# MarvinChung/simple-implementation-of-structure-from-motion-and-multi-view-stereo-by-python

Measured on AMD Instinct MI355X. Metric: candidate patches/sec NCC-scored (640×480, 48 views) at 1/2/4/8 MI355X; % HBM roofline, higher is better.
Workload: dtype u8; 1 GPU; dinoRing 48x640x480, one expansion sweep of 1048576 candidates per GPU, 11x11 NCC (wid=5) vs all views, MIN_NCC 0.7, one GPU (no exchange); global_batch=1048576, wid=5, views=48, outputs=per candidate: xy + one record [mask word, avg] (|V| = popcount), parallelism=single GPU

## Files before the change

include/mvs_amd.h:

```cpp
#ifndef MVS_AMD_H
#define MVS_AMD_H

#include <stdint.h>

#ifdef __cplusplus
extern "C" {
#endif

#define MVS_OK 0
#define MVS_E_ARG (-1)
#define MVS_E_HIP (-2)
#define MVS_E_UNSUPPORTED (-3)
#define MVS_E_NOMEM (-4)
#define MVS_E_DIVZERO (-5)

typedef struct mvs_ctx mvs_ctx;
typedef struct mvs_stage_result mvs_stage_result;
typedef struct mvs_stage mvs_stage;

const char* mvs_version(void);

int mvs_ctx_create(int device, int V, int H, int W, const uint8_t* rgb, const double* K,
                   const double* R, const double* t, const double* Rp, mvs_ctx** out);
void mvs_ctx_destroy(mvs_ctx* ctx);
// ... 19 lines not shown
                        const uint64_t* mask, const int32_t* count, const double* avg,
                        const double* c, const double* nrm, uint8_t* alive, int64_t* stats);
int mvs_pack_accepted(mvs_ctx* ctx, int64_t n, int64_t offset, const int32_t* d_count,
                      const uint64_t* d_mask, const double* d_c, int vlb, int64_t cap, int64_t* d_out,
                      void* stream);
int mvs_proxy_copy(void* d_dst, const void* d_src, int64_t bytes, int workgroups, void* stream);
int mvs_set_scorer_grid(mvs_ctx* ctx, int workgroups);
int mvs_kernel_timing(mvs_ctx* ctx, int enable);
int mvs_kernel_time(mvs_ctx* ctx, double* total_ms, int64_t* launches);
const char* mvs_timed_kernel(const mvs_ctx* ctx);
int64_t mvs_exact_hits(mvs_ctx* ctx);
int mvs_stream_retiring(mvs_ctx* ctx, void* stream);

int mvs_scorer_stats(mvs_ctx* ctx, int64_t* out);

int mvs_ncc_windows(int64_t n, int npx, const uint8_t* d_a, const uint8_t* d_b, double thr,
                    int force_exact, double* d_ncc, uint8_t* d_pass, void* stream);

int mvs_stage_run(mvs_ctx* ctx, int64_t n_tracks, const int64_t* track_off,
                  const int32_t* obs_view, const float* obs_xy, int cell_size, double scale,
                  int wid, int64_t max_pops, mvs_stage_result** out);
int64_t mvs_stage_count(const mvs_stage_result* res, int which);
int mvs_stage_rows(const mvs_stage_result* res, int which, double* rows);
int mvs_stage_rows_device(const mvs_stage_result* res, int which, double* d_rows, void* stream);
int mvs_stage_stats(const mvs_stage_result* res, int64_t* stats);
int mvs_stage_times(const mvs_stage_result* res, double* times);
void mvs_stage_free(mvs_stage_result* res);

#define MVS_STAGE_FILTER_OUTLIERS 1
int mvs_exact_avg(mvs_ctx* ctx, int64_t n, const int32_t* ref, const double* xy, const uint64_t* mask,
// ... 40 lines not shown
```

simple-implementation-of-structure-from-motion-and-multi-view-stereo-by-python_amd/_lib.py:

```python
import atexit
import ctypes
import os
import weakref

import numpy as np

HERE = os.path.dirname(os.path.abspath(__file__))
LIB_PATH = os.path.join(HERE, "libmvs_amd.so")

_dp = ctypes.POINTER(ctypes.c_double)
_fp = ctypes.POINTER(ctypes.c_float)
_u8p = ctypes.POINTER(ctypes.c_uint8)
_i32p = ctypes.POINTER(ctypes.c_int32)
_i64p = ctypes.POINTER(ctypes.c_int64)
_u64p = ctypes.POINTER(ctypes.c_uint64)
_vp = ctypes.c_void_p

SIGNATURES = [
    ("mvs_version", ctypes.c_char_p, []),
    ("mvs_last_error", ctypes.c_char_p, [_vp]),
    ("mvs_ctx_create", ctypes.c_int, [ctypes.c_int, ctypes.c_int, ctypes.c_int, ctypes.c_int, _u8p,
                                      _dp, _dp, _dp, _dp, ctypes.POINTER(_vp)]),
    ("mvs_ctx_destroy", None, [_vp]),
    ("mvs_ctx_rproj", ctypes.c_int, [_vp, _dp]),
# ... 4 lines not shown
                                        ctypes.c_double, _vp, _vp, _vp, _vp, _vp]),
    ("mvs_score_device_rec", ctypes.c_int, [_vp, ctypes.c_int64, _vp, _vp, ctypes.c_int, ctypes.c_double,
                                            _vp, _vp, _vp]),
    ("mvs_score_warped", ctypes.c_int, [_vp, ctypes.c_int64, _dp, _dp, _i32p, ctypes.c_int, ctypes.c_double,
                                        ctypes.c_double, _dp, _u64p, _i32p, _dp, _dp]),
    ("mvs_score_warped_device", ctypes.c_int, [_vp, ctypes.c_int64, _vp, _vp, _vp, ctypes.c_int,
                                               ctypes.c_double, ctypes.c_double, _vp, _vp, _vp, _vp, _vp, _vp]),
    ("mvs_pack_accepted", ctypes.c_int, [_vp, ctypes.c_int64, ctypes.c_int64, _vp, _vp, _vp, ctypes.c_int,
                                         ctypes.c_int64, _vp, _vp]),
    ("mvs_set_scorer_grid", ctypes.c_int, [_vp, ctypes.c_int]),
    ("mvs_proxy_copy", ctypes.c_int, [_vp, _vp, ctypes.c_int64, ctypes.c_int, _vp]),
    ("mvs_filter_outliers", ctypes.c_int, [ctypes.c_int64, ctypes.c_int, ctypes.c_int, ctypes.c_int, _i32p,
                                           _u64p, _i32p, _dp, _dp, _dp, _u8p, _i64p]),
    ("mvs_exact_hits", ctypes.c_int64, [_vp]),
    ("mvs_scorer_stats", ctypes.c_int, [_vp, _i64p]),
    ("mvs_stream_retiring", ctypes.c_int, [_vp, _vp]),
    ("mvs_kernel_timing", ctypes.c_int, [_vp, ctypes.c_int]),
    ("mvs_kernel_time", ctypes.c_int, [_vp, ctypes.POINTER(ctypes.c_double),
                                       ctypes.POINTER(ctypes.c_int64)]),
    ("mvs_timed_kernel", ctypes.c_char_p, [_vp]),
    ("mvs_ncc_windows", ctypes.c_int, [ctypes.c_int64, ctypes.c_int, _vp, _vp, ctypes.c_double,
                                       ctypes.c_int, _vp, _vp, _vp]),
    ("mvs_stage_run", ctypes.c_int, [_vp, ctypes.c_int64, _i64p, _i32p, _fp, ctypes.c_int,
                                     ctypes.c_double, ctypes.c_int, ctypes.c_int64,
                                     ctypes.POINTER(_vp)]),
    ("mvs_stage_begin", ctypes.c_int, [_vp, ctypes.c_int64, _i64p, _i32p, _fp, ctypes.c_int,
                                       ctypes.c_double, ctypes.c_int, ctypes.c_int64, ctypes.c_int,
                                       ctypes.c_int, ctypes.POINTER(_vp)]),
    ("mvs_stage_plan", ctypes.c_int64, [_vp]),
    ("mvs_stage_record_width", ctypes.c_int, [_vp]),
# ... 189 lines not shown
        return self._h

    def rproj(self):
        out = np.empty((self.V, 9))
        check(load().mvs_ctx_rproj(self._h, _p(out, _dp)), self._h, "mvs_ctx_rproj")
        return out.reshape(self.V, 3, 3)

    def exact_hits(self):
        return int(load().mvs_exact_hits(self._h))

    def scorer_stats(self):
        out = np.zeros(3, np.int64)
        check(load().mvs_scorer_stats(self._h, _p(out, _i64p)), self._h, "mvs_scorer_stats")
        return {"direct": int(out[0]), "overflow": int(out[1]), "batches": int(out[2])}

    def rebuild(self, stream=None):
        check(load().mvs_ctx_rebuild(self._h, stream), self._h, "mvs_ctx_rebuild")

    def kernel_timing(self, enable=True, every=1):
        check(load().mvs_kernel_timing(self._h, int(every) if enable else 0), self._h, "mvs_kernel_timing")

    def kernel_time(self):
        ms = ctypes.c_double(0.0)
        k = ctypes.c_int64(0)
        check(load().mvs_kernel_time(self._h, ctypes.byref(ms), ctypes.byref(k)), self._h,
              "mvs_kernel_time")
        return ms.value, int(k.value)

    def timed_kernel(self):
        name = load().mvs_timed_kernel(self._h)
# ... 280 lines not shown
```

simple-implementation-of-structure-from-motion-and-multi-view-stereo-by-python_amd/csrc/mvs_engine.cpp:

```cpp
#include <algorithm>
#include <chrono>
#include <cfloat>
#include <cmath>
#include <cstdio>
#include <cstdlib>
#include <cstring>
#include <memory>
#include <string>
#include <vector>

#include "../../include/mvs_amd.h"
#include "mvs_internal.h"

namespace {

thread_local std::string g_err;

struct Fail {
    int code;
    std::string msg;
};

#define HIPCHK(x)                                                                         \
    do {                                                                                  \
// ... 240 lines not shown
    std::vector<uint8_t> h_rgb;
    DevBuf<uint8_t> d_rgb, d_stack, d_gv;
    DevBuf<CamDev> d_cams;
    DevBuf<int32_t> d_exact;
    DevBuf<unsigned long long> d_stats;
    SceneDev sc{};
    DevBuf<double> s_c, s_xy, s_avg;
    DevBuf<int32_t> s_ref, s_count;
    DevBuf<uint64_t> s_mask;
    DevBuf<double> w_in, w_out, w_ncc;
    DevBuf<int32_t> w_ref, w_count;
    DevBuf<uint64_t> w_mask;
    DevBuf<int32_t> t_tiles, t_cand;
    DevBuf<unsigned long long> p_ctl;
    DevBuf<int4> t_items;
    DevBuf<float> f_resp, f_dil;
    DevBuf<uint32_t> f_key, f_desc;
    DevBuf<int32_t> f_rows, f_pts, f_mom, f_best;
    int kernel_mode = 0;
    int tab_mode = 0;
    int scorer_wgs = 0;
    DevBuf<int16_t> mom_sb[MVS_MAX_WID + 1];
    DevBuf<double> mom_w[MVS_MAX_WID + 1];
    DevBuf<int32_t> mom_d[MVS_MAX_WID + 1];
    DevBuf<uint16_t> mom_flat[MVS_MAX_WID + 1];
    bool mom_ok[MVS_MAX_WID + 1] = {};
    int moments_vp() const { return V > MVS_GROUP_VIEWS ? 64 * ((V + 63) / 64) : 16 * ((V + 15) / 16); }
    MomentsDev moments(int wid) const {
        MomentsDev m{};
        m.sb = mom_sb[wid].p;
// ... 159 lines not shown
    a.xy = d_xy;
    a.mask = d_mask;
    a.count = d_count;
    a.avg = d_avg;
    a.exact_hits = ctx->d_exact.p;
    a.mstride = ctx->words();
    a.astride = 1;
    a.rec = 0;
    if (!d_count) {
        a.rec = 1;
        a.mstride = a.astride = ctx->words() + 1;
        a.avg = (double*)(d_mask + ctx->words());
    }
    const bool grouped = ctx->V > MVS_GROUP_VIEWS;
    const bool tiled = ctx->kernel_mode == 2 || (ctx->kernel_mode == 0 && n >= 2048);
    if (tiled) {
        TiledArgs t{};
        t.tw = MVS_TILE_W;
        t.th = MVS_TILE_H;
        t.ntx = (ctx->W + MVS_TILE_W - 1) / MVS_TILE_W;
        t.nty = (ctx->H + MVS_TILE_H - 1) / MVS_TILE_H;
        const int ntiles = t.ntx * t.nty;
        const int32_t* tiles_before = ctx->t_tiles.p;
        const int64_t set_words = tc_words(ntiles);
        ctx->t_tiles.ensure((size_t)(2 * set_words));
        if (ctx->t_tiles.p != tiles_before) ctx->tiles_clean_ntiles = -1;
        const int groups = grouped ? (ctx->V + MVS_GROUP_VIEWS - 1) / MVS_GROUP_VIEWS : 1;
        const int64_t mean = (n + ntiles - 1) / ntiles;
        int64_t cap = std::min<int64_t>(std::max<int64_t>(16 * mean, 1024), std::max<int64_t>(n, 64));
        cap = (cap + 63) & ~(int64_t)63;
// ... 8 lines not shown
        t.tile_count = set;
        int32_t* ctl = set + (int64_t)ntiles * kTcStride;
        t.head = ctl;
        t.fix_count = ctl + 32;
        t.n_items = ctl + 96;
        t.zero_blk = ctx->t_tiles.p + (1 - ctx->tiles_parity) * set_words;
        t.zero_words = set_words;
        t.sorted = (int2*)ctx->t_cand.p;
        t.fix_list = (int4*)(ctx->t_cand.p + 2 * (size_t)ntiles * cap);
        t.item_seg = (int)(n / std::max(t.chunk, 1) + ntiles + 2);
        ctx->t_items.ensure((size_t)kItemSegs * t.item_seg);
        t.items = ctx->t_items.p;
        t.zero_first = ctx->tiles_clean_ntiles != ntiles ? 1 : 0;
        t.grid = ctx->scorer_wgs;
        t.stats = ctx->d_stats.p;
        ctx->tiles_clean_ntiles = -1;
        hipEvent_t e0, e1;
        ctx->next_events(&e0, &e1);
        ctx->scratch_acquire(s);
        const bool tab = ctx->ensure_moments(wid, s);
        const MomentsDev mt = ctx->moments(wid);
        const int rc = mvs_launch_score_tiled(&ctx->sc, &a, &t, wid, tab ? &mt : nullptr, s, e0, e1);
        if (rc != 0) throw Fail{rc == -3 ? MVS_E_UNSUPPORTED : MVS_E_HIP, "tiled score launch failed"};
        ctx->scratch_release(s);
        if (e0) ctx->timed_name = mvs_timed_kernel_name(ctx->V, wid, tab && !grouped ? 2 : 1);
        ctx->tiles_clean_ntiles = ntiles;
        ctx->tiles_parity ^= 1;
        return;
    }
    hipEvent_t e0, e1;
    ctx->next_events(&e0, &e1);
    if (mvs_launch_score(&ctx->sc, &a, wid, s, e0, e1) != 0) throw Fail{MVS_E_HIP, "score launch failed"};
    if (e0) ctx->timed_name = mvs_timed_kernel_name(ctx->V, wid, 0);
}

void expand_device(mvs_ctx* ctx, const RecordsDev& r, const ExpandArgs& a, int wid, hipStream_t s) {
// ... 707 lines not shown
        HIPCHK(hipMemcpyAsync(ctx->d_cams.p, ctx->cams.data(), V * sizeof(CamDev), hipMemcpyHostToDevice, ctx->stream));
        ctx->d_exact.alloc(1);
        HIPCHK(hipMemsetAsync(ctx->d_exact.p, 0, sizeof(int32_t), ctx->stream));
        ctx->d_stats.alloc(4);
        HIPCHK(hipMemsetAsync(ctx->d_stats.p, 0, 4 * sizeof(unsigned long long), ctx->stream));
        HIPCHK(hipStreamSynchronize(ctx->stream));
        ctx->sc.cams = ctx->d_cams.p;
        if (const char* km = std::getenv("MVS_SCORE_KERNEL")) {
            if (!std::strcmp(km, "direct")) ctx->kernel_mode = 1;
            else if (!std::strcmp(km, "tiled")) ctx->kernel_mode = 2;
            else if (!std::strcmp(km, "mma")) ctx->tab_mode = 1;
            else if (!std::strcmp(km, "tab")) ctx->tab_mode = 2;
        }
        if (const char* sw = std::getenv("MVS_SCORER_WGS")) ctx->scorer_wgs = std::max(0, std::atoi(sw));
        if (const char* tl = std::getenv("MVS_TAB_LIMIT")) ctx->tab_limit = std::max<int64_t>(1, std::atoll(tl));
        return 0;
    });
    if (rc != 0) {
        g_err = ctx->err;
        return rc;
    }
    *out = ctx.release();
    return 0;
}

void mvs_ctx_destroy(mvs_ctx* ctx) {
    if (!ctx) return;
    (void)hipSetDevice(ctx->device);
    if (ctx->scratch_order.used || ctx->pack_order.used) (void)hipDeviceSynchronize();
    if (ctx->stream) (void)hipStreamSynchronize(ctx->stream);
// ... 250 lines not shown
        ctx->pack_order.retire((hipStream_t)stream);
        return 0;
    });
}

int mvs_scorer_stats(mvs_ctx* ctx, int64_t* out) {
    if (!ctx || !out) return set_err(ctx, Fail{MVS_E_ARG, "null argument"});
    return guarded(ctx, [&]() {
        unsigned long long h[4] = {0, 0, 0, 0};
        HIPCHK(hipMemcpyAsync(h, ctx->d_stats.p, sizeof h, hipMemcpyDeviceToHost, ctx->stream));
        HIPCHK(hipStreamSynchronize(ctx->stream));
        for (int k = 0; k < 3; ++k) out[k] = (int64_t)h[k];
        return 0;
    });
}

int mvs_ncc_windows(int64_t n, int npx, const uint8_t* d_a, const uint8_t* d_b, double thr,
                    int force_exact, double* d_ncc, uint8_t* d_pass, void* stream) {
    if (npx < 1 || npx > 128) return set_err(nullptr, Fail{MVS_E_UNSUPPORTED, "npx must be in 1..128"});
    int rc = mvs_launch_ncc_windows(n, npx, d_a, d_b, thr, force_exact, d_ncc, d_pass, (hipStream_t)stream);
    if (rc) return set_err(nullptr, Fail{MVS_E_HIP, "ncc_windows launch failed"});
    return 0;
}

int mvs_stage_run(mvs_ctx* ctx, int64_t n_tracks, const int64_t* track_off, const int32_t* obs_view,
                  const float* obs_xy, int cell_size, double scale, int wid, int64_t max_pops,
                  mvs_stage_result** out) {
    if (!ctx) return set_err(nullptr, Fail{MVS_E_ARG, "null context"});
    if (!out || n_tracks < 0 || (n_tracks > 0 && (!track_off || !obs_view || !obs_xy)) || cell_size < 1)
        return set_err(ctx, Fail{MVS_E_ARG, "bad arguments"});
// ... 447 lines not shown
```

simple-implementation-of-structure-from-motion-and-multi-view-stereo-by-python_amd/csrc/mvs_internal.h:

```cpp
#pragma once
#include <hip/hip_runtime.h>
#include <stdint.h>

#define MVS_MAX_VIEWS 256
#define MVS_MAX_WID 5

struct CamDev {
    double Rp[9];
    double t[3];
    double fx, fy, cx, cy;
    double R[9];
    double O[3];
    double C[3];
    double fbar;
    double pad[3];
};

struct SceneDev {
    int V, H, W;
    int Wq;
    int64_t row_bytes;
    const uint8_t* stack;
    const uint8_t* rgb;
    const CamDev* cams;
// ... 47 lines not shown
    int32_t* tile_count;
    int32_t* head;
    int2* sorted;
    int4* fix_list;
    int32_t* fix_count;
    int32_t* n_items;
    int item_seg;
    int32_t* zero_blk;
    int64_t zero_words;
    int groups;
    int zero_first;
    int4* items;
    int grid;
    int implicit;
    unsigned long long* stats;
};
#ifndef MVS_BIN_PER
#define MVS_BIN_PER 4
#endif
#ifndef MVS_BIN_BLOCK
#define MVS_BIN_BLOCK 1024
#endif
#define MVS_BIN_CHUNK (MVS_BIN_BLOCK * MVS_BIN_PER)
struct MomentsDev {
    int16_t* sb;
    double* w;
    int32_t* d;
    uint16_t* flat;
    int VP;
    int wid;
};
// ... 33 lines not shown
#define MVS_GROUP_VIEWS 64
#define MVS_GROUP_CHUNK 116
#ifndef MVS_ACC_PER
#define MVS_ACC_PER 8
#endif
#define MVS_ACC_CHUNK (1024 * MVS_ACC_PER)

extern "C" {
int mvs_launch_build_scene(const SceneDev* sc, const uint8_t* d_rgb, uint8_t* d_stack, uint8_t* d_gv_base,
                           hipStream_t s);
int mvs_launch_score(const SceneDev* sc, const ScoreArgs* a, int wid, hipStream_t s,
                     hipEvent_t ev0, hipEvent_t ev1);
int mvs_launch_score_warp(const SceneDev* sc, const WarpArgs* a, int wid, hipStream_t s);
int mvs_launch_score_tiled(const SceneDev* sc, const ScoreArgs* a, const TiledArgs* t, int wid,
                           const MomentsDev* mt, hipStream_t s, hipEvent_t ev0, hipEvent_t ev1);
int mvs_launch_moments(const SceneDev* sc, const MomentsDev* mt, hipStream_t s);
int mvs_launch_score_tab(const SceneDev* sc, const ScoreArgs* a, const TiledArgs* t, const MomentsDev* mt,
                         hipStream_t s);
size_t mvs_mma_lds_bytes(int V, int wid);
const char* mvs_timed_kernel_name(int V, int wid, int tiled);
int mvs_launch_expand(const SceneDev* sc, RecordsDev rec, const ExpandArgs* a, int wid,
                      hipStream_t s);
int mvs_launch_expand_geom(const SceneDev* sc, RecordsDev rec, const ExpandArgs* a, hipStream_t s);
int mvs_launch_expand_accept(RecordsDev rec, const ExpandArgs* a, hipStream_t s);
int mvs_launch_expand_ingest(RecordsDev rec, const ExpandArgs* a, int words, hipStream_t s);
int mvs_launch_pack_accepted(int64_t n, int64_t offset, const int32_t* count, const uint64_t* mask, const double* c,
                             int words, int vlb, int64_t cap, unsigned long long* ctl, int64_t* out, hipStream_t s);
int mvs_launch_proxy_copy(void* dst, const void* src, int64_t bytes, int workgroups, hipStream_t s);
int mvs_launch_ncc_windows(int64_t n, int npx, const uint8_t* a, const uint8_t* b, double thr,
                           int force_exact, double* ncc, uint8_t* pass, hipStream_t s);
// ... 19 lines not shown
```

simple-implementation-of-structure-from-motion-and-multi-view-stereo-by-python_amd/csrc/mvs_kernels.hip:

```cpp
#include <algorithm>
#include <atomic>
#include <cstdlib>
#include <utility>

#include <hipcub/hipcub.hpp>

#include "mvs_device.h"
#include "mvs_mma.h"

namespace {

template <int WID>
__device__ __noinline__ double exact_ncc_stack(const SceneDev sc, int R, int v, int q, int r) {
    constexpr int NB = 2 * WID + 1, NPX = NB * NB;
    constexpr int NW = (NB + 3) / 4, ND = NW + 1;
    const int64_t vstride = (int64_t)sc.V * 4;
    const int o = (q - WID) & 3;
    const uint8_t* p0 = sc.stack + (int64_t)(r - WID) * sc.row_bytes + (int64_t)((q - WID) >> 2) * vstride;
    auto window = [&](int view, uint32_t (&w)[NB][NW]) {
        uint32_t d[NB][ND];
#pragma unroll
        for (int row = 0; row < NB; ++row)
#pragma unroll
            for (int j = 0; j < ND; ++j)
// ... 327 lines not shown
    __syncthreads();
    if (threadIdx.x == 0) {
        int run = 0;
        for (int w = 0; w < kScanThreads / 64; ++w) { const int c = s_w[w]; s_w[w] = run; run += c; }
        s_w[kScanThreads / 64] = run;
    }
    __syncthreads();
    int slot = s_w[threadIdx.x >> 6] + incl - mine;
    for (int k = t0; k < t1; ++k) {
        const int c = min(t.tile_count[k * kTcStride], t.cap);
        for (int j = 0; j * t.chunk < c; ++j) t.items[slot++] = make_int4(k, j, 0, 0);
    }
    if (threadIdx.x < kItemSegs) t.n_items[32 * threadIdx.x] = threadIdx.x == 0 ? s_w[kScanThreads / 64] : 0;
}

template <bool LDSHIST>
__global__ __launch_bounds__(kBinBlock) void k_bin(const SceneDev sc, const ScoreArgs a,
                                                   const TiledArgs t, int wid, const MomentsDev mt) {
    extern __shared__ int32_t hist[];
    __shared__ double s_cam[16][MVS_MAX_VIEWS];
    const int words = (sc.V + 63) >> 6;
    const int64_t base = (int64_t)blockIdx.x * kBinBlock * kBinPer;
    int Rk[kBinPer];
    double ck[kBinPer][3];
#pragma unroll
    for (int k = 0; k < kBinPer; ++k) {
        const int64_t i = base + (int64_t)k * kBinBlock + threadIdx.x;
        const int64_t ii = i < a.n ? i : 0;
        Rk[k] = a.ref[ii];
        ck[k][0] = a.c[3 * ii];
        ck[k][1] = a.c[3 * ii + 1];
// ... 57 lines not shown
        }
        const int R = Rk[k], q = qk[k], r = rk[k];
        const int tx = q / MVS_TILE_W, ty = r / MVS_TILE_H;
        const int tile = ty * t.ntx + tx;
        tl[k] = tile;
        pk[k] = (q - tx * MVS_TILE_W) | ((r - ty * MVS_TILE_H) << 4) | (R << 7);
        if (LDSHIST) {
            lr[k] = atomicAdd(&hist[tile], 1);
        } else {
            lr[k] = atomicAdd(&t.tile_count[tile * kTcStride], 1);
            if (t.implicit && lr[k] > 0 && lr[k] < t.cap && lr[k] % t.chunk == 0)
                t.items[t.item_seg + atomicAdd(&t.n_items[32], 1)] = make_int4(tile, lr[k] / t.chunk, 0, 0);
        }
    }
    STAMP(t1);
    if (LDSHIST) {
        __syncthreads();
        int bs[kBinLdsTiles / kBinBlock];
#pragma unroll
        for (int j = 0; j < kBinLdsTiles / kBinBlock; ++j) {
            const int b = threadIdx.x + j * kBinBlock;
            const int c = b < t.ntiles ? hist[b] : 0;
            bs[j] = c ? atomicAdd(&t.tile_count[b * kTcStride], c) : 0;
        }
        auto bs_tile = [&](int jj) { return (int)threadIdx.x + jj * kBinBlock; };
        if (t.implicit) {
#pragma unroll
            for (int j = 0; j < kBinLdsTiles / kBinBlock; ++j) {
                const int b = bs_tile(j);
                const int c = b < t.ntiles ? hist[b] : 0;
// ... 1555 lines not shown
                         hipStream_t s, hipEvent_t ev0, hipEvent_t ev1) {
    if (a->n == 0) return 0;
    const bool grouped = sc->V > kGroupViews;
    if (t->tw != MVS_TILE_W || t->th != MVS_TILE_H || t->items == nullptr ||
        t->chunk != (grouped ? kGroupChunk : kMmaChunk) || t->groups != (grouped ? (sc->V + 63) / 64 : 1) ||
        sc->V > MVS_MAX_VIEWS)
        return -3;
    if (t->zero_first &&
        (hipMemsetAsync(t->tile_count, 0, sizeof(int32_t) * tc_words(t->ntiles), s) != hipSuccess ||
         hipMemsetAsync(t->zero_blk, 0, sizeof(int32_t) * t->zero_words, s) != hipSuccess))
        return -1;
    const int64_t per_block = (int64_t)kBinBlock * kBinPer;
    const int nbin = (int)((a->n + per_block - 1) / per_block);
    TiledArgs tv = *t;
    tv.implicit = (!grouped && mt && a->n >= (int64_t)kImplicitMean * t->ntiles) ? 1 : 0;
    const MomentsDev mflat = mt ? *mt : MomentsDev{};
    if (t->ntiles <= kBinLdsTiles)
        hipLaunchKernelGGL(k_bin<true>, dim3(nbin), dim3(kBinBlock), (size_t)t->ntiles * 4, s, *sc, *a, tv, WID, mflat);
    else
        hipLaunchKernelGGL(k_bin<false>, dim3(nbin), dim3(kBinBlock), 0, s, *sc, *a, tv, WID, mflat);
    if (!tv.implicit) hipLaunchKernelGGL(k_item_scan, dim3(1), dim3(kScanThreads), 0, s, tv);
    t = &tv;
    int rc = 0;
    {
        TimedLaunch tl(s, ev0, ev1);
        if (grouped) rc = launch_mma<WID, 4, true>(sc, a, t, mt, s);
        else if (mt) rc = mvs_launch_score_tab(sc, a, t, mt, s);
        else switch ((sc->V + 15) / 16) {
            case 1: rc = launch_mma<WID, 1, false>(sc, a, t, nullptr, s); break;
            case 2: rc = launch_mma<WID, 2, false>(sc, a, t, nullptr, s); break;
            case 3: rc = launch_mma<WID, 3, false>(sc, a, t, nullptr, s); break;
            default: rc = launch_mma<WID, 4, false>(sc, a, t, nullptr, s); break;
// ... 25 lines not shown
    return hipGetLastError() == hipSuccess ? 0 : -1;
}

int grid_for(int64_t n, int block, int cap) {
    return (int)std::max<int64_t>(1, std::min<int64_t>((n + block - 1) / block, cap));
}

}

#ifdef MVS_STAMPS
extern "C" int mvs_read_stamps(unsigned long long* out) {
    return hipMemcpyFromSymbol(out, HIP_SYMBOL(g_stamps), sizeof(g_stamps)) == hipSuccess ? 0 : -1;
}
#endif

extern "C" int mvs_launch_build_scene(const SceneDev* sc, const uint8_t* d_rgb, uint8_t* d_stack,
                                      uint8_t* d_gv_base, hipStream_t s) {
    (void)d_gv_base;
    const dim3 grid((unsigned)((sc->W + kSceneStrip - 1) / kSceneStrip), (unsigned)sc->H);
    hipLaunchKernelGGL(k_build_scene, grid, dim3(256), 0, s, *sc, d_rgb, d_stack, (uint8_t*)sc->gv);
    return hipGetLastError() == hipSuccess ? 0 : -1;
}

extern "C" int mvs_launch_score(const SceneDev* sc, const ScoreArgs* a, int wid, hipStream_t s,
                                hipEvent_t ev0, hipEvent_t ev1) {
    switch (wid) {
        case 1: return launch_score_w<1>(sc, a, s, ev0, ev1);
        case 2: return launch_score_w<2>(sc, a, s, ev0, ev1);
        case 3: return launch_score_w<3>(sc, a, s, ev0, ev1);
        case 4: return launch_score_w<4>(sc, a, s, ev0, ev1);
// ... 143 lines not shown
```

simple-implementation-of-structure-from-motion-and-multi-view-stereo-by-python_amd/csrc/mvs_score_tab.hip:

```cpp
#include <algorithm>

#include "mvs_device.h"
#include "mvs_mma.h"

namespace {

constexpr int kMomW = 32, kMomH = 16, kMomV = 16;

template <int WID, bool DTAB>
__global__ __launch_bounds__(256) void k_moments(const SceneDev sc, const MomentsDev mt) {
    constexpr int NB = 2 * WID + 1, NPX = NB * NB;
    constexpr int ROWS = kMomH + 2 * WID, CP = 48, CW = CP / 4, GP = CW + 1;
    __shared__ __attribute__((aligned(16))) uint32_t g4[kMomV][ROWS][GP];
    const int x0 = blockIdx.x * kMomW, y0 = blockIdx.y * kMomH, v0 = blockIdx.z * kMomV;
    const int tid = threadIdx.x;
    const int nv = min(kMomV, sc.V - v0);
    constexpr int NLD = kMomV * ROWS * CW, PER = (NLD + 255) / 256;
    uint32_t buf[PER];
#pragma unroll
    for (int j = 0; j < PER; ++j) {
        const int k = tid + 256 * j;
        const int vi = k / (ROWS * CW), rc = k - vi * (ROWS * CW), r = rc / CW, c = rc - r * CW;
        const int y = min(max(y0 - WID + r, 0), sc.H - 1);
        uint32_t wv = 0u;
// ... 73 lines not shown
            }
        }
    }
}

#ifdef MVS_STAMPS
__device__ unsigned long long g_stamps_tab[1024 * 16];
#define TSTAMP(var) const unsigned long long var = __builtin_amdgcn_s_memtime()
#define TSTAMP_ADD(slot, val) \
    do { if ((threadIdx.x & 63) == 0) atomicAdd(&g_stamps_tab[(blockIdx.x & 1023) * 16 + (slot)], (unsigned long long)(val)); } while (0)
#else
#define TSTAMP(var)
#define TSTAMP_ADD(slot, val)
#endif

constexpr int kTabWaves = 8, kTabThreads = 64 * kTabWaves, kTabGrid = 512;
constexpr int kTabBudget = 80 * 1024 - 512;
constexpr int kTabMinWaves = (2 * kTabWaves + 3) / 4;
constexpr int kTabChunk = MVS_MMA_CHUNK;

struct alignas(16) TabInfo {
    int32_t tix;
    int32_t Sa;
    int32_t R;
    float T;
};

template <int WID, int NBLK>
struct TabGeom {
    static constexpr int VP = 16 * NBLK;
    static constexpr int RB = VP * MmaGeom<WID>::VS;
    static constexpr int CB = kTabChunk * 8;
    static constexpr int FIXED = kTabWaves * 32 * (int)sizeof(TabInfo) + 65 * 8 + 64;
    static constexpr int BUF = (RB + 16) + CB;
    static_assert(BUF + FIXED <= kTabBudget, "one item's buffers fit");
    static constexpr bool DB = 2 * BUF + FIXED <= kTabBudget;
};

template <int WID, int NBLK, bool FAST>
__global__ __launch_bounds__(kTabThreads, kTabMinWaves) void k_score_tab(const SceneDev sc, const ScoreArgs a, const TiledArgs t,
                                                               const MomentsDev mt, const int4* __restrict__ items,
                                                               const int2* __restrict__ sorted) {
    using G = MmaGeom<WID>;
    using TG = TabGeom<WID, NBLK>;
    constexpr int NB = G::NB, NPX = G::NPX, KS = G::KS, VS = G::VS, C0 = G::C0;
    constexpr int VP = TG::VP;
    constexpr bool DB = TG::DB;

    constexpr int RPV = VS / 32;
    constexpr int PF = (VP * RPV * 2 + kTabThreads - 1) / kTabThreads;
    constexpr int RB = TG::RB, CB = TG::CB;
    __shared__ __attribute__((aligned(16))) uint8_t s_reg0[RB + 16], s_reg1[DB ? RB + 16 : 16];
    __shared__ __attribute__((aligned(16))) uint8_t s_cand0[CB], s_cand1[DB ? CB : 16];
    __shared__ __attribute__((aligned(16))) TabInfo s_ti[kTabWaves * 32];
    __shared__ int s_ids[2];
    __shared__ double s_recip[65];
#ifdef MVS_STAMPS
    const unsigned long long t_wg0 = __builtin_amdgcn_s_memrealtime();
#endif
    const int tid = threadIdx.x, lane = tid & 63;
    const int wave = __builtin_amdgcn_readfirstlane(tid >> 6);
    const int V = sc.V;
    const int npiece = V * RPV * 2;
    if (tid <= 64) s_recip[tid] = c_recip.r[tid];
    if (tid < 4) ((uint32_t*)(s_reg0 + RB))[tid] = 0u;
    if (DB && tid >= 4 && tid < 8) ((uint32_t*)(s_reg1 + RB))[tid & 3] = 0u;
    TabInfo* ti = s_ti + wave * 32;

    const double kn = (double)NPX / (double)(NPX - 1);
    const float tqf = (float)(a.thr / kn);
    ItemMap im;
    im.load(t);
    const bool implicit = t.implicit != 0;
    const int n_units = implicit ? t.ntiles + t.n_items[32] : im.total();
    int32_t* head = t.head;
    const int16_t* __restrict__ tsb = mt.sb;
    const double* __restrict__ tw = mt.w;

    auto region_buf = [&](auto bufc) -> uint8_t* { return decltype(bufc)::value ? s_reg1 : s_reg0; };
    auto cand_buf = [&](auto bufc) -> uint8_t* { return decltype(bufc)::value ? s_cand1 : s_cand0; };
    auto stage = [&](const int4 d, auto bufc) {
        const int ty = d.x / t.ntx, tx = d.x - ty * t.ntx;
        const int x0 = tx * MVS_TILE_W, yr0 = ty * MVS_TILE_H - WID;
        uint8_t* base = region_buf(bufc);
#pragma unroll
        for (int p = 0; p < PF; ++p) {
            const int k = opaque(tid) + p * kTabThreads;
            const int v = k / (2 * RPV), r2 = k - v * (2 * RPV);
            if (k < npiece && (r2 >> 1) != RPV - 1) {
// ... 4 lines not shown
                                                 16, 0, 0);
            }
        }
        uint8_t* cbase = cand_buf(bufc);
        const uint8_t* csrc = (const uint8_t*)(sorted + d.y);
#pragma unroll
        for (int p = 0; p < (kTabChunk / 2 + kTabThreads - 1) / kTabThreads; ++p) {
            const int k = tid + p * kTabThreads;
            if (k < d.w / 2)
                __builtin_amdgcn_global_load_lds((const void*)(csrc + 16 * k),
                                                 (void __attribute__((address_space(3)))*)(cbase + (p * kTabThreads + wave * 64) * 16),
                                                 16, 0, 0);
        }
    };

    constexpr int kBands = kBandHeads;
    const int ob = (int)blockIdx.x % kBands;
    int32_t* bheads = head + (3 + kItemSegs) * 32;
    auto bstart = [&](int x) -> int { return (int)((int64_t)n_units * x / kBands); };
    auto bwgs = [&](int x) -> int { return ((int)gridDim.x - x + kBands - 1) / kBands; };
    int cb = ob;
    auto claim = [&]() -> int {
        return band_claim(bheads, cb, ob, kBands, n_units, [&](int x) { return 2 * bwgs(x); });
    };
    auto desc = [&](int2 it, int cnt) -> int4 {
        const int tile = __builtin_amdgcn_readfirstlane(it.x), j = __builtin_amdgcn_readfirstlane(it.y);
        const int c = __builtin_amdgcn_readfirstlane(cnt);
        return make_int4(tile, tile * t.cap + j * t.chunk, min(min(c, t.cap) - j * t.chunk, t.chunk),
                         min(t.chunk, t.cap - j * t.chunk));
    };
// ... 5 lines not shown
    if (tid == 0) {
        const int l = (int)blockIdx.x / kBands, bs = bstart(ob), bn = bstart(ob + 1) - bs;
        const int s0 = l < bn ? bs + l : -1, s1 = l + bwgs(ob) < bn ? bs + l + bwgs(ob) : -1;
        const int c0 = s0 >= 0 ? s0 : claim();
        s_ids[0] = c0;
        s_ids[1] = s1 >= 0 ? s1 : c0 < n_units ? claim() : n_units;
    }
    __syncthreads();
    int cur = __builtin_amdgcn_readfirstlane(s_ids[0]);
    int nx1 = __builtin_amdgcn_readfirstlane(s_ids[1]);
    if (cur >= n_units) return;
    int4 dcur;
    {
        const int2 it = implicit && cur < t.ntiles ? make_int2(cur, 0) : item_v(cur);
        const int tile = __builtin_amdgcn_readfirstlane(it.x), j = __builtin_amdgcn_readfirstlane(it.y);
        stage(make_int4(tile, tile * t.cap + j * t.chunk, 0, min(t.chunk, t.cap - j * t.chunk)),
              std::integral_constant<int, 0>{});
        dcur = desc(it, count_v(it.x));
    }
    int2 it1 = make_int2(0, 0);
    int pend = nx1;
    __syncthreads();

    auto round = [&](auto bufc) -> bool {
        constexpr int buf = decltype(bufc)::value;
        const int nc = dcur.z;
        const uint8_t* reg = region_buf(bufc);
        int2* cand = (int2*)cand_buf(bufc);
        const int zoff = RB;
        TSTAMP(ts0);
        if (tid == 0) s_ids[0] = pend;
        asm volatile("s_waitcnt vmcnt(0)" ::: "memory");
        __syncthreads();
        TSTAMP(ts1);
        nx1 = __builtin_amdgcn_readfirstlane(s_ids[0]);
        if (nx1 < n_units) {
            const int2 iv = item_v(nx1);
            it1 = make_int2(__builtin_amdgcn_readfirstlane(iv.x), __builtin_amdgcn_readfirstlane(iv.y));
        }
        const int j1 = it1.y;
        const int4 dst1 = make_int4(it1.x, it1.x * t.cap + j1 * t.chunk, 0, min(t.chunk, t.cap - j1 * t.chunk));
        if constexpr (DB) {
            if (nx1 < n_units) stage(dst1, std::integral_constant<int, buf ^ 1>{});
        }
        const int c1 = count_v(it1.x);
        TSTAMP(ts1b);
        TSTAMP_ADD(7, ts1b - ts1);
        const int ty = dcur.x / t.ntx, tx = dcur.x - ty * t.ntx;
        const int tix0 = ((ty * MVS_TILE_H) * sc.W + tx * MVS_TILE_W) * VP;
        const int nblk = (nc + 15) >> 4;
        const int b0 = nblk * wave / kTabWaves, b1 = nblk * (wave + 1) / kTabWaves;
        {
            const int base = 16 * b0, cnt = min(16 * b1, nc) - base;
            constexpr int SH = 5, NBINS = 4;
            int2 e0 = make_int2(0, 0), e1 = make_int2(0, 0);
            int bin0 = NBINS, bin1 = NBINS;
            if (lane < cnt) { e0 = cand[base + lane]; bin0 = (e0.y >> SH) & (NBINS - 1); }
            if (lane + 64 < cnt) { e1 = cand[base + 64 + lane]; bin1 = (e1.y >> SH) & (NBINS - 1); }
            int r0 = 0, r1 = 0, run = 0;
            static_for<NBINS>([&](auto Yc) {
// ... 242 lines not shown
                                                                     (uint32_t)(ab >> 32));
                        } else {
                            a.mask[idx] = mk;
                            a.count[idx] = cnt;
                            if (a.avg) a.avg[idx] = av;
                        }
                        if (gg) t.fix_list[atomicAdd(t.fix_count, 1)] = make_int4((int32_t)idx, dcur.x, e[h].y, 0);
                    }
                }
                TSTAMP(tk2);
                TSTAMP_ADD(6, tk2 - tk1);
            };
            if (nh == 2) unit(std::integral_constant<int, 2>{});
            else unit(std::integral_constant<int, 1>{});
            TSTAMP_ADD(4, nh);
            if (fb == b0 && tid == 0 && nx1 < n_units) pend = claim();
        }
        if (b0 >= b1 && tid == 0 && nx1 < n_units) pend = claim();
        TSTAMP(ts3);
        if (wave == 0) TSTAMP_ADD(0, 1);
        TSTAMP_ADD(1, ts1 - ts0);
        TSTAMP_ADD(2, ts2 - ts1);
        TSTAMP_ADD(3, ts3 - ts2);
        if (nx1 >= n_units) return false;
        if constexpr (!DB) {
            __syncthreads();
            stage(dst1, std::integral_constant<int, 0>{});
        }
        cur = nx1;
        dcur = desc(it1, c1);
        return true;
    };
    for (;;) {
        if (!round(std::integral_constant<int, 0>{})) break;
        if (!round(std::integral_constant<int, DB ? 1 : 0>{})) break;
    }
#ifdef MVS_STAMPS
    if (tid == 0) {
        atomicAdd(&g_stamps_tab[(blockIdx.x & 1023) * 16 + 10], (unsigned long long)t_wg0);
        atomicAdd(&g_stamps_tab[(blockIdx.x & 1023) * 16 + 11], (unsigned long long)__builtin_amdgcn_s_memrealtime());
        const unsigned hw = __builtin_amdgcn_s_getreg((31 << 11) | (0 << 6) | 4);
        const unsigned xcc = __builtin_amdgcn_s_getreg((15 << 11) | (0 << 6) | 20);
        atomicAdd(&g_stamps_tab[(blockIdx.x & 1023) * 16 + 12], (unsigned long long)hw + 1ull);
        atomicAdd(&g_stamps_tab[(blockIdx.x & 1023) * 16 + 13], (unsigned long long)xcc + 1ull);
    }
#endif
}


template <int WID, int NBLK>
int launch_tab(const SceneDev* sc, const ScoreArgs* a, const TiledArgs* t, const MomentsDev* mt, hipStream_t s) {
    const dim3 grid(t->grid > 0 ? std::min(t->grid, kTabGrid) : kTabGrid);
    if (fabs(a->thr) >= 0.01)
        hipLaunchKernelGGL((k_score_tab<WID, NBLK, true>), grid, dim3(kTabThreads), 0, s, *sc, *a, *t, *mt,
                           (const int4*)t->items, (const int2*)t->sorted);
    else
        hipLaunchKernelGGL((k_score_tab<WID, NBLK, false>), grid, dim3(kTabThreads), 0, s, *sc, *a, *t, *mt,
                           (const int4*)t->items, (const int2*)t->sorted);
    return hipGetLastError() == hipSuccess ? 0 : -1;
}

template <int WID>
int launch_tab_w(const SceneDev* sc, const ScoreArgs* a, const TiledArgs* t, const MomentsDev* mt, hipStream_t s) {
    switch ((sc->V + 15) / 16) {
        case 1: return launch_tab<WID, 1>(sc, a, t, mt, s);
        case 2: return launch_tab<WID, 2>(sc, a, t, mt, s);
        case 3: return launch_tab<WID, 3>(sc, a, t, mt, s);
        default: return launch_tab<WID, 4>(sc, a, t, mt, s);
    }
}

}

// ... 42 lines not shown
```

Before: 10.29 billion candidates/s.

## Bin candidates into per-block sorted runs and gather them in the scorer

The binning kernel gains a runs mode. Each bin block scans its LDS tile histogram and writes its candidates sorted by tile into a per-block run, along with a uint16 offset table. The scorer no longer reads globally atomically binned tile lists. It gathers each tile's candidates from up to 256 block runs with wave prefix scans, pipelining the gather with the double-buffered staging and sending overflow past the tile capacity to the fix list. This aims to remove the global atomic scatter and the separate item compaction, at the cost of extra offset-table reads and gather logic in the scorer.

```diff
diff --git a/include/mvs_amd.h b/include/mvs_amd.h
--- a/include/mvs_amd.h
+++ b/include/mvs_amd.h
@@ -57,6 +57,8 @@
 
 int mvs_scorer_stats(mvs_ctx* ctx, int64_t* out);
 
+int64_t mvs_bin_runs_batches(mvs_ctx* ctx);
+
 int mvs_ncc_windows(int64_t n, int npx, const uint8_t* d_a, const uint8_t* d_b, double thr,
                     int force_exact, double* d_ncc, uint8_t* d_pass, void* stream);
 
diff --git a/simple-implementation-of-structure-from-motion-and-multi-view-stereo-by-python_amd/_lib.py b/simple-implementation-of-structure-from-motion-and-multi-view-stereo-by-python_amd/_lib.py
--- a/simple-implementation-of-structure-from-motion-and-multi-view-stereo-by-python_amd/_lib.py
+++ b/simple-implementation-of-structure-from-motion-and-multi-view-stereo-by-python_amd/_lib.py
@@ -42,6 +42,7 @@
                                            _u64p, _i32p, _dp, _dp, _dp, _u8p, _i64p]),
     ("mvs_exact_hits", ctypes.c_int64, [_vp]),
     ("mvs_scorer_stats", ctypes.c_int, [_vp, _i64p]),
+    ("mvs_bin_runs_batches", ctypes.c_int64, [_vp]),
     ("mvs_stream_retiring", ctypes.c_int, [_vp, _vp]),
     ("mvs_kernel_timing", ctypes.c_int, [_vp, ctypes.c_int]),
     ("mvs_kernel_time", ctypes.c_int, [_vp, ctypes.POINTER(ctypes.c_double),
@@ -261,6 +262,9 @@
         check(load().mvs_scorer_stats(self._h, _p(out, _i64p)), self._h, "mvs_scorer_stats")
         return {"direct": int(out[0]), "overflow": int(out[1]), "batches": int(out[2])}
 
+    def bin_runs_batches(self):
+        return int(load().mvs_bin_runs_batches(self._h))
+
     def rebuild(self, stream=None):
         check(load().mvs_ctx_rebuild(self._h, stream), self._h, "mvs_ctx_rebuild")
 
diff --git a/simple-implementation-of-structure-from-motion-and-multi-view-stereo-by-python_amd/csrc/mvs_engine.cpp b/simple-implementation-of-structure-from-motion-and-multi-view-stereo-by-python_amd/csrc/mvs_engine.cpp
--- a/simple-implementation-of-structure-from-motion-and-multi-view-stereo-by-python_amd/csrc/mvs_engine.cpp
+++ b/simple-implementation-of-structure-from-motion-and-multi-view-stereo-by-python_amd/csrc/mvs_engine.cpp
@@ -278,6 +278,10 @@
     DevBuf<int32_t> t_tiles, t_cand;
     DevBuf<unsigned long long> p_ctl;
     DevBuf<int4> t_items;
+    DevBuf<int2> t_runs;
+    DevBuf<uint16_t> t_offs;
+    int runs_max = kRunsLimit;
+    int64_t runs_batches = 0;
     DevBuf<float> f_resp, f_dil;
     DevBuf<uint32_t> f_key, f_desc;
     DevBuf<int32_t> f_rows, f_pts, f_mom, f_best;
@@ -467,6 +471,7 @@
     }
     const bool grouped = ctx->V > MVS_GROUP_VIEWS;
     const bool tiled = ctx->kernel_mode == 2 || (ctx->kernel_mode == 0 && n >= 2048);
+    if (tiled && n == 0) return;
     if (tiled) {
         TiledArgs t{};
         t.tw = MVS_TILE_W;
@@ -505,12 +510,21 @@
         t.zero_first = ctx->tiles_clean_ntiles != ntiles ? 1 : 0;
         t.grid = ctx->scorer_wgs;
         t.stats = ctx->d_stats.p;
+        const int64_t nbin = (n + MVS_BIN_CHUNK - 1) / MVS_BIN_CHUNK;
+        t.runs_max = std::min(ctx->runs_max, kRunsLimit);
+        if (nbin <= t.runs_max) {
+            ctx->t_runs.ensure((size_t)nbin * MVS_BIN_CHUNK);
+            ctx->t_offs.ensure((size_t)nbin * (ntiles + 1));
+            t.runs = ctx->t_runs.p;
+            t.offs = ctx->t_offs.p;
+        }
         ctx->tiles_clean_ntiles = -1;
         hipEvent_t e0, e1;
         ctx->next_events(&e0, &e1);
         ctx->scratch_acquire(s);
         const bool tab = ctx->ensure_moments(wid, s);
         const MomentsDev mt = ctx->moments(wid);
+        if (mvs_tiled_uses_runs(&ctx->sc, &a, &t, tab ? &mt : nullptr)) ++ctx->runs_batches;
         const int rc = mvs_launch_score_tiled(&ctx->sc, &a, &t, wid, tab ? &mt : nullptr, s, e0, e1);
         if (rc != 0) throw Fail{rc == -3 ? MVS_E_UNSUPPORTED : MVS_E_HIP, "tiled score launch failed"};
         ctx->scratch_release(s);
@@ -1248,6 +1262,9 @@
         }
         if (const char* sw = std::getenv("MVS_SCORER_WGS")) ctx->scorer_wgs = std::max(0, std::atoi(sw));
         if (const char* tl = std::getenv("MVS_TAB_LIMIT")) ctx->tab_limit = std::max<int64_t>(1, std::atoll(tl));
+        if (const char* rm = std::getenv("MVS_BIN_RUNS_MAX")) ctx->runs_max = std::min(std::max(0, std::atoi(rm)), kRunsLimit);
+        if (const char* bm = std::getenv("MVS_BIN"))
+            if (!std::strcmp(bm, "atomic")) ctx->runs_max = 0;
         return 0;
     });
     if (rc != 0) {
@@ -1528,6 +1545,8 @@
         return 0;
     });
 }
+
+int64_t mvs_bin_runs_batches(mvs_ctx* ctx) { return ctx ? ctx->runs_batches : 0; }
 
 int mvs_ncc_windows(int64_t n, int npx, const uint8_t* d_a, const uint8_t* d_b, double thr,
                     int force_exact, double* d_ncc, uint8_t* d_pass, void* stream) {
diff --git a/simple-implementation-of-structure-from-motion-and-multi-view-stereo-by-python_amd/csrc/mvs_internal.h b/simple-implementation-of-structure-from-motion-and-multi-view-stereo-by-python_amd/csrc/mvs_internal.h
--- a/simple-implementation-of-structure-from-motion-and-multi-view-stereo-by-python_amd/csrc/mvs_internal.h
+++ b/simple-implementation-of-structure-from-motion-and-multi-view-stereo-by-python_amd/csrc/mvs_internal.h
@@ -85,7 +85,13 @@
     int grid;
     int implicit;
     unsigned long long* stats;
+    int2* runs;
+    uint16_t* offs;
+    int runs_max;
+    int use_runs;
+    int nbin;
 };
+constexpr int kRunsLimit = 256;
 #ifndef MVS_BIN_PER
 #define MVS_BIN_PER 4
 #endif
@@ -149,6 +155,7 @@
 int mvs_launch_score_warp(const SceneDev* sc, const WarpArgs* a, int wid, hipStream_t s);
 int mvs_launch_score_tiled(const SceneDev* sc, const ScoreArgs* a, const TiledArgs* t, int wid,
                            const MomentsDev* mt, hipStream_t s, hipEvent_t ev0, hipEvent_t ev1);
+int mvs_tiled_uses_runs(const SceneDev* sc, const ScoreArgs* a, const TiledArgs* t, const MomentsDev* mt);
 int mvs_launch_moments(const SceneDev* sc, const MomentsDev* mt, hipStream_t s);
 int mvs_launch_score_tab(const SceneDev* sc, const ScoreArgs* a, const TiledArgs* t, const MomentsDev* mt,
                          hipStream_t s);
diff --git a/simple-implementation-of-structure-from-motion-and-multi-view-stereo-by-python_amd/csrc/mvs_kernels.hip b/simple-implementation-of-structure-from-motion-and-multi-view-stereo-by-python_amd/csrc/mvs_kernels.hip
--- a/simple-implementation-of-structure-from-motion-and-multi-view-stereo-by-python_amd/csrc/mvs_kernels.hip
+++ b/simple-implementation-of-structure-from-motion-and-multi-view-stereo-by-python_amd/csrc/mvs_kernels.hip
@@ -365,7 +365,7 @@
     if (threadIdx.x < kItemSegs) t.n_items[32 * threadIdx.x] = threadIdx.x == 0 ? s_w[kScanThreads / 64] : 0;
 }
 
-template <bool LDSHIST>
+template <bool LDSHIST, bool RUNS = false>
 __global__ __launch_bounds__(kBinBlock) void k_bin(const SceneDev sc, const ScoreArgs a,
                                                    const TiledArgs t, int wid, const MomentsDev mt) {
     extern __shared__ int32_t hist[];
@@ -453,6 +453,52 @@
         }
     }
     STAMP(t1);
+    if constexpr (RUNS) {
+        static_assert(LDSHIST, "the runs come from the LDS histogram");
+        __shared__ int s_w[kBinBlock / 64];
+        __syncthreads();
+        const int per = (t.ntiles + kBinBlock - 1) / kBinBlock;
+        const int k0 = min((int)threadIdx.x * per, t.ntiles), k1 = min(k0 + per, t.ntiles);
+        int mine = 0;
+        for (int k = k0; k < k1; ++k) mine += hist[k];
+        int incl = mine;
+#pragma unroll
+        for (int d = 1; d < 64; d <<= 1) {
+            const int o = __shfl_up(incl, d, 64);
+            if ((threadIdx.x & 63) >= d) incl += o;
+        }
+        if ((threadIdx.x & 63) == 63) s_w[threadIdx.x >> 6] = incl;
+        __syncthreads();
+        int run = incl - mine, total = 0;
+#pragma unroll
+        for (int w = 0; w < kBinBlock / 64; ++w) {
+            const int c = s_w[w];
+            if (w < (int)(threadIdx.x >> 6)) run += c;
+            total += c;
+        }
+        for (int k = k0; k < k1; ++k) {
+            const int c = hist[k];
+            hist[k] = run;
+            run += c;
+        }
+        __syncthreads();
+        STAMP(t2);
+        uint16_t* orow = t.offs + (int64_t)blockIdx.x * (t.ntiles + 1);
+        for (int k = threadIdx.x; k <= t.ntiles; k += kBinBlock) orow[k] = (uint16_t)(k < t.ntiles ? hist[k] : total);
+        int2* myrun = t.runs + (int64_t)blockIdx.x * MVS_BIN_CHUNK;
+#pragma unroll
+        for (int k = 0; k < kBinPer; ++k) {
+            const int64_t i = base + (int64_t)k * kBinBlock + threadIdx.x;
+            if (tl[k] < 0) continue;
+            myrun[hist[tl[k]] + lr[k]] = make_int2((int32_t)i, pk[k]);
+        }
+        STAMP(t3);
+        STAMP_ADD_ROW(2048 + blockIdx.x, 0, 1);
+        STAMP_ADD_ROW(2048 + blockIdx.x, 1, t1 - t0);
+        STAMP_ADD_ROW(2048 + blockIdx.x, 2, t2 - t1);
+        STAMP_ADD_ROW(2048 + blockIdx.x, 3, t3 - t2);
+        return;
+    }
     if (LDSHIST) {
         __syncthreads();
         int bs[kBinLdsTiles / kBinBlock];
@@ -2038,8 +2084,12 @@
     const int nbin = (int)((a->n + per_block - 1) / per_block);
     TiledArgs tv = *t;
     tv.implicit = (!grouped && mt && a->n >= (int64_t)kImplicitMean * t->ntiles) ? 1 : 0;
+    tv.nbin = nbin;
+    tv.use_runs = mvs_tiled_uses_runs(sc, a, t, mt);
     const MomentsDev mflat = mt ? *mt : MomentsDev{};
-    if (t->ntiles <= kBinLdsTiles)
+    if (tv.use_runs)
+        hipLaunchKernelGGL((k_bin<true, true>), dim3(nbin), dim3(kBinBlock), (size_t)t->ntiles * 4, s, *sc, *a, tv, WID, mflat);
+    else if (t->ntiles <= kBinLdsTiles)
         hipLaunchKernelGGL(k_bin<true>, dim3(nbin), dim3(kBinBlock), (size_t)t->ntiles * 4, s, *sc, *a, tv, WID, mflat);
     else
         hipLaunchKernelGGL(k_bin<false>, dim3(nbin), dim3(kBinBlock), 0, s, *sc, *a, tv, WID, mflat);
@@ -2095,6 +2145,13 @@
 }
 #endif
 
+extern "C" int mvs_tiled_uses_runs(const SceneDev* sc, const ScoreArgs* a, const TiledArgs* t, const MomentsDev* mt) {
+    const int64_t nbin = (a->n + MVS_BIN_CHUNK - 1) / MVS_BIN_CHUNK;
+    const bool dense = sc->V <= kGroupViews && mt && a->n >= (int64_t)kImplicitMean * t->ntiles;
+    const bool fits = t->ntiles <= kBinLdsTiles && nbin <= std::min(t->runs_max, kRunsLimit);
+    return dense && a->n > 0 && fits && t->runs && t->offs ? 1 : 0;
+}
+
 extern "C" int mvs_launch_build_scene(const SceneDev* sc, const uint8_t* d_rgb, uint8_t* d_stack,
                                       uint8_t* d_gv_base, hipStream_t s) {
     (void)d_gv_base;
diff --git a/simple-implementation-of-structure-from-motion-and-multi-view-stereo-by-python_amd/csrc/mvs_score_tab.hip b/simple-implementation-of-structure-from-motion-and-multi-view-stereo-by-python_amd/csrc/mvs_score_tab.hip
--- a/simple-implementation-of-structure-from-motion-and-multi-view-stereo-by-python_amd/csrc/mvs_score_tab.hip
+++ b/simple-implementation-of-structure-from-motion-and-multi-view-stereo-by-python_amd/csrc/mvs_score_tab.hip
@@ -111,6 +111,22 @@
 #define TSTAMP_ADD(slot, val)
 #endif
 
+DEV int wave_sum(int x) {
+#pragma unroll
+    for (int off = 32; off > 0; off >>= 1) x += __shfl_xor(x, off, 64);
+    return x;
+}
+
+DEV int wave_scan_add(int x) {
+    x += __builtin_amdgcn_update_dpp(0, x, 0x111, 0xf, 0xf, false);
+    x += __builtin_amdgcn_update_dpp(0, x, 0x112, 0xf, 0xf, false);
+    x += __builtin_amdgcn_update_dpp(0, x, 0x114, 0xf, 0xf, false);
+    x += __builtin_amdgcn_update_dpp(0, x, 0x118, 0xf, 0xf, false);
+    x += __builtin_amdgcn_update_dpp(0, x, 0x142, 0xa, 0xf, false);
+    x += __builtin_amdgcn_update_dpp(0, x, 0x143, 0xc, 0xf, false);
+    return x;
+}
+
 constexpr int kTabWaves = 8, kTabThreads = 64 * kTabWaves, kTabGrid = 512;
 constexpr int kTabBudget = 80 * 1024 - 512;
 constexpr int kTabMinWaves = (2 * kTabWaves + 3) / 4;
@@ -134,7 +150,7 @@
     static constexpr bool DB = 2 * BUF + FIXED <= kTabBudget;
 };
 
-template <int WID, int NBLK, bool FAST>
+template <int WID, int NBLK, bool FAST, bool RUNS>
 __global__ __launch_bounds__(kTabThreads, kTabMinWaves) void k_score_tab(const SceneDev sc, const ScoreArgs a, const TiledArgs t,
                                                                const MomentsDev mt, const int4* __restrict__ items,
                                                                const int2* __restrict__ sorted) {
@@ -151,6 +167,7 @@
     __shared__ __attribute__((aligned(16))) uint8_t s_cand0[CB], s_cand1[DB ? CB : 16];
     __shared__ __attribute__((aligned(16))) TabInfo s_ti[kTabWaves * 32];
     __shared__ int s_ids[2];
+    __shared__ int s_tot[2];
     __shared__ double s_recip[65];
 #ifdef MVS_STAMPS
     const unsigned long long t_wg0 = __builtin_amdgcn_s_memrealtime();
@@ -167,9 +184,10 @@
     const double kn = (double)NPX / (double)(NPX - 1);
     const float tqf = (float)(a.thr / kn);
     ItemMap im;
-    im.load(t);
-    const bool implicit = t.implicit != 0;
-    const int n_units = implicit ? t.ntiles + t.n_items[32] : im.total();
+    if constexpr (!RUNS) im.load(t);
+    const bool implicit = RUNS || t.implicit != 0;
+    const int n_units = RUNS ? t.ntiles : implicit ? t.ntiles + t.n_items[32] : im.total();
+    constexpr bool runs = RUNS;
     int32_t* head = t.head;
     const int16_t* __restrict__ tsb = mt.sb;
     const double* __restrict__ tw = mt.w;
@@ -204,6 +222,95 @@
         }
     };
 
+    constexpr bool DEFER = DB && NBLK < 4;
+    constexpr int GUP = 3;
+    struct Gath {
+        uint32_t r[2 * GUP + 2];
+    };
+    static_assert(kRunsLimit / 64 <= 2 * GUP + 2, "the count columns fit the register set");
+    const int g_waves = (t.nbin + 63) >> 6;
+    auto g_issue = [&](int tile, Gath& g) {
+        if (wave >= g_waves) return;
+        const uint16_t* __restrict__ offs = t.offs;
+        const int ol = opaque(lane);
+#pragma unroll
+        for (int jj = 0; jj < kRunsLimit / 64; ++jj) {
+            g.r[jj] = 0u;
+            if (jj <= wave) {
+                const int k = min(64 * jj + ol, t.nbin - 1) * (t.ntiles + 1) + tile;
+                __builtin_memcpy(&g.r[jj], offs + k, 4);
+            }
+        }
+    };
+    auto g_scan = [&](int tile, int j, Gath& g, auto bufc) {
+        constexpr int buf = decltype(bufc)::value;
+        if (wave >= g_waves) return;
+        const int2* __restrict__ rsrc = t.runs;
+        const int ol = opaque(lane);
+        int low = 0, cnt = 0, o0 = 0;
+#pragma unroll
+        for (int jj = 0; jj < kRunsLimit / 64; ++jj) {
+            const int a0 = (int)(g.r[jj] & 0xffffu), a1 = (int)(g.r[jj] >> 16);
+            const int c = 64 * jj + ol < t.nbin ? a1 - a0 : 0;
+            if (jj < wave) low += c;
+            if (jj == wave) { cnt = c; o0 = a0; }
+        }
+        const int pre = __builtin_amdgcn_readlane(wave_scan_add(low), 63);
+        const int incl = wave_scan_add(cnt);
+        const int rank0 = pre + incl - cnt;
+        if (wave == g_waves - 1 && ol == 63) s_tot[buf] = pre + incl;
+        const int lo = j * t.chunk, hi = min(lo + t.chunk, t.cap);
+        const int e0 = max(lo - rank0, 0), e1 = min(cnt, hi - rank0);
+        const int sb = (64 * wave + ol) * MVS_BIN_CHUNK + o0;
+        const int n = max(e1 - e0, 0);
+        g.r[2 * GUP] = (uint32_t)((n << 16) | (n ? rank0 - lo + e0 : 0));
+        g.r[2 * GUP + 1] = (uint32_t)(sb + e0);
+        if (n) {
+#pragma unroll
+            for (int u = 0; u < GUP; ++u) {
+                const int2 v = rsrc[sb + e0 + min(u, n - 1)];
+                g.r[2 * u] = (uint32_t)v.x;
+                g.r[2 * u + 1] = (uint32_t)v.y;
+            }
+        }
+        if (j == 0) {
+            const int f0 = max(t.cap - rank0, 0);
+            const int ov = max(cnt - f0, 0);
+            uint64_t om = __ballot(ov > 0);
+            if (om) {
+                int slot = 0;
+                if (ov > 0) slot = atomicAdd(t.fix_count, ov);
+                if (t.stats) {
+                    const int tot = wave_sum(ov);
+                    if (ol == 0) atomicAdd(&t.stats[1], (unsigned long long)tot);
+                }
+                for (; om; om &= om - 1) {
+                    const int l = __builtin_ctzll(om);
+                    const int n_l = __builtin_amdgcn_readlane(ov, l);
+                    const int src_l = __builtin_amdgcn_readlane(sb + f0, l);
+                    const int slot_l = __builtin_amdgcn_readlane(slot, l);
+                    for (int e = ol; e < n_l; e += 64) {
+                        const int2 v = rsrc[src_l + e];
+                        t.fix_list[slot_l + e] = make_int4(v.x, tile, v.y, 0);
+                    }
+                }
+            }
+        }
+    };
+    auto g_write = [&](const Gath& g, auto bufc) {
+        if (wave >= g_waves) return;
+        const int n = (int)(g.r[2 * GUP] >> 16);
+        int2* dst = (int2*)cand_buf(bufc) + (g.r[2 * GUP] & 0xffffu);
+        if (n) {
+#pragma unroll
+            for (int u = 0; u < GUP; ++u)
+                if (u < n) dst[u] = make_int2((int)g.r[2 * u], (int)g.r[2 * u + 1]);
+            const int2* __restrict__ rsrc = t.runs;
+            const int src = (int)g.r[2 * GUP + 1];
+            for (int e = GUP; e < n; ++e) dst[e] = rsrc[src + e];
+        }
+    };
+
     constexpr int kBands = kBandHeads;
     const int ob = (int)blockIdx.x % kBands;
     int32_t* bheads = head + (3 + kItemSegs) * 32;
@@ -239,17 +346,24 @@
     {
         const int2 it = implicit && cur < t.ntiles ? make_int2(cur, 0) : item_v(cur);
         const int tile = __builtin_amdgcn_readfirstlane(it.x), j = __builtin_amdgcn_readfirstlane(it.y);
-        stage(make_int4(tile, tile * t.cap + j * t.chunk, 0, min(t.chunk, t.cap - j * t.chunk)),
+        stage(make_int4(tile, tile * t.cap + j * t.chunk, 0, runs ? 0 : min(t.chunk, t.cap - j * t.chunk)),
               std::integral_constant<int, 0>{});
-        dcur = desc(it, count_v(it.x));
-    }
+        if constexpr (runs) {
+            Gath g;
+            g_issue(tile, g);
+            g_scan(tile, 0, g, std::integral_constant<int, 0>{});
+            g_write(g, std::integral_constant<int, 0>{});
+        }
+        dcur = desc(it, runs ? 0 : count_v(it.x));
+    }
+    int curj = 0;
     int2 it1 = make_int2(0, 0);
     int pend = nx1;
     __syncthreads();
 
     auto round = [&](auto bufc) -> bool {
         constexpr int buf = decltype(bufc)::value;
-        const int nc = dcur.z;
+        int nc = dcur.z;
         const uint8_t* reg = region_buf(bufc);
         int2* cand = (int2*)cand_buf(bufc);
         const int zoff = RB;
@@ -259,16 +373,35 @@
         __syncthreads();
         TSTAMP(ts1);
         nx1 = __builtin_amdgcn_readfirstlane(s_ids[0]);
-        if (nx1 < n_units) {
+        bool more = false;
+        if (runs) {
+            const int below = min(__builtin_amdgcn_readfirstlane(s_tot[buf]), t.cap);
+            nc = max(min(below - curj * t.chunk, t.chunk), 0);
+            more = (curj + 1) * t.chunk < below;
+        }
+        if (more) {
+            it1 = make_int2(dcur.x, curj + 1);
+        } else if (nx1 < n_units) {
             const int2 iv = item_v(nx1);
             it1 = make_int2(__builtin_amdgcn_readfirstlane(iv.x), __builtin_amdgcn_readfirstlane(iv.y));
         }
         const int j1 = it1.y;
-        const int4 dst1 = make_int4(it1.x, it1.x * t.cap + j1 * t.chunk, 0, min(t.chunk, t.cap - j1 * t.chunk));
+        const int4 dst1 = make_int4(it1.x, it1.x * t.cap + j1 * t.chunk, 0,
+                                    runs ? 0 : min(t.chunk, t.cap - j1 * t.chunk));
+        const bool nextv = nx1 < n_units || more;
+        Gath g;
         if constexpr (DB) {
-            if (nx1 < n_units) stage(dst1, std::integral_constant<int, buf ^ 1>{});
-        }
-        const int c1 = count_v(it1.x);
+            if (nextv) {
+                if constexpr (runs) g_issue(it1.x, g);
+                if constexpr (runs && !DEFER) {
+                    g_scan(it1.x, j1, g, std::integral_constant<int, buf ^ 1>{});
+                    g_write(g, std::integral_constant<int, buf ^ 1>{});
+                }
+                stage(dst1, std::integral_constant<int, buf ^ 1>{});
+            }
+        }
+        int c1 = 0;
+        if constexpr (!runs) c1 = count_v(it1.x);
         TSTAMP(ts1b);
         TSTAMP_ADD(7, ts1b - ts1);
         const int ty = dcur.x / t.ntx, tx = dcur.x - ty * t.ntx;
@@ -541,19 +674,37 @@
             if (nh == 2) unit(std::integral_constant<int, 2>{});
             else unit(std::integral_constant<int, 1>{});
             TSTAMP_ADD(4, nh);
-            if (fb == b0 && tid == 0 && nx1 < n_units) pend = claim();
-        }
-        if (b0 >= b1 && tid == 0 && nx1 < n_units) pend = claim();
+            if (fb == b0 && tid == 0 && nx1 < n_units && !more) pend = claim();
+            if constexpr (runs && DEFER) {
+                if (fb == b0 && nextv) g_scan(it1.x, j1, g, std::integral_constant<int, buf ^ 1>{});
+            }
+        }
+        if (b0 >= b1 && tid == 0 && nx1 < n_units && !more) pend = claim();
+        if constexpr (runs && DEFER) {
+            if (b0 >= b1 && nextv) g_scan(it1.x, j1, g, std::integral_constant<int, buf ^ 1>{});
+            if (nextv) g_write(g, std::integral_constant<int, buf ^ 1>{});
+        }
         TSTAMP(ts3);
         if (wave == 0) TSTAMP_ADD(0, 1);
         TSTAMP_ADD(1, ts1 - ts0);
         TSTAMP_ADD(2, ts2 - ts1);
         TSTAMP_ADD(3, ts3 - ts2);
-        if (nx1 >= n_units) return false;
+        if (nx1 >= n_units && !more) return false;
         if constexpr (!DB) {
             __syncthreads();
+            if constexpr (runs) {
+                Gath g0;
+                g_issue(it1.x, g0);
+                g_scan(it1.x, j1, g0, std::integral_constant<int, 0>{});
+                g_write(g0, std::integral_constant<int, 0>{});
+            }
             stage(dst1, std::integral_constant<int, 0>{});
         }
+        if (more) {
+            ++curj;
+            return true;
+        }
+        curj = 0;
         cur = nx1;
         dcur = desc(it1, c1);
         return true;
@@ -578,12 +729,18 @@
 template <int WID, int NBLK>
 int launch_tab(const SceneDev* sc, const ScoreArgs* a, const TiledArgs* t, const MomentsDev* mt, hipStream_t s) {
     const dim3 grid(t->grid > 0 ? std::min(t->grid, kTabGrid) : kTabGrid);
-    if (fabs(a->thr) >= 0.01)
-        hipLaunchKernelGGL((k_score_tab<WID, NBLK, true>), grid, dim3(kTabThreads), 0, s, *sc, *a, *t, *mt,
-                           (const int4*)t->items, (const int2*)t->sorted);
-    else
-        hipLaunchKernelGGL((k_score_tab<WID, NBLK, false>), grid, dim3(kTabThreads), 0, s, *sc, *a, *t, *mt,
-                           (const int4*)t->items, (const int2*)t->sorted);
+#define MVS_TAB_LAUNCH(FAST_, RUNS_)                                                                            \
+    hipLaunchKernelGGL((k_score_tab<WID, NBLK, FAST_, RUNS_>), grid, dim3(kTabThreads), 0, s, *sc, *a, *t, *mt, \
+                       (const int4*)t->items, (const int2*)t->sorted)
+    const bool fast = fabs(a->thr) >= 0.01;
+    if (t->use_runs) {
+        if (fast) MVS_TAB_LAUNCH(true, true);
+        else MVS_TAB_LAUNCH(false, true);
+    } else {
+        if (fast) MVS_TAB_LAUNCH(true, false);
+        else MVS_TAB_LAUNCH(false, false);
+    }
+#undef MVS_TAB_LAUNCH
     return hipGetLastError() == hipSuccess ? 0 : -1;
 }
 
```

New measurement: 10.82 billion candidates/s (median of 6 runs). 1.05x the previous value.
